# smdogroup/eigd

Measured on AMD Instinct MI355X. Metric: adjoint_mode_derivatives_per_sec, higher is better.
Workload: dtype f64

## Files before the change

### eigd_amd/_ffi.py

```python

import ctypes as C
import os

import numpy as np

_HERE = os.path.dirname(os.path.abspath(__file__))
LIB_PATH = os.environ.get("EIGD_LIB") or os.path.join(_HERE, "lib", "libeigd_hip.so")

EIGD_E_INVALID, EIGD_E_HIP, EIGD_E_NOTSPD, EIGD_E_INTERNAL = -1, -2, -3, -4


class EigdHipError(RuntimeError):
    """HIP runtime / device failure inside libeigd_hip.so."""


class NotPositiveDefiniteError(np.linalg.LinAlgError):
    """The shifted matrix handed to SpLuOperator is not positive definite."""


_lib = None

c_int, c_i64, c_dbl, c_sz, c_vp = C.c_int, C.c_int64, C.c_double, C.c_size_t, C.c_void_p
P = C.POINTER

# ... 52 lines not shown
    "eigd_project_stats": [c_vp, c_vp],
    "eigd_svqb_step": [c_vp, c_int, c_int, c_vp, c_int, c_vp, c_int, c_vp, c_int, c_vp, c_int],
    "eigd_project_to": [c_vp, c_int, c_int, c_int, c_vp, c_int, c_vp, c_int, c_vp, c_int, c_vp, c_int, c_dbl, c_vp, c_vp],
    "eigd_coldot_dev": [c_vp, c_int, c_int, c_vp, c_int, c_vp, c_int, c_vp],
    "eigd_coldot": [c_vp, c_int, c_int, c_vp, c_int, c_vp, c_int, c_vp],
    "eigd_coldot_dd": [c_vp, c_int, c_int, c_vp, c_int, c_vp, c_int, c_vp],
    "eigd_lincomb": [c_vp, c_int, c_int, c_vp, c_int, c_int, c_vp, c_vp, c_vp],
    "eigd_stack_dot": [c_vp, c_int, c_int, c_int, c_vp, c_i64, c_int, c_vp, c_int, c_vp],
    "eigd_stack_axpy": [c_vp, c_int, c_int, c_int, c_vp, c_i64, c_int, c_vp, c_vp, c_int, c_dbl],
    "eigd_stack_axpy_dot": [c_vp, c_int, c_int, c_int, c_vp, c_i64, c_int, c_vp, c_vp, c_int, c_dbl, c_vp],
    "eigd_stack_cgs2": [c_vp, c_int, c_int, c_int, c_vp, c_i64, c_int, c_vp, c_int, c_dbl, c_vp, c_vp],
    "eigd_stack_cgs2_pair": [c_vp, c_int, c_int, c_int, c_vp, c_i64, c_int, c_vp, c_int, c_dbl, c_vp, c_vp],
    "eigd_pair_orthonormalise": [c_vp, c_int, c_int, c_vp, c_int, c_vp, c_vp, c_int, c_vp, c_int, c_vp, c_vp],
    "eigd_csr_update_values_dev": [c_vp, c_vp],
    "eigd_factor_refactor_dev": [c_vp, c_vp],
    "eigd_assembler_create": [c_vp, c_int, c_int, c_int, c_vp, c_vp],
    "eigd_assembler_free": [c_vp],
    "eigd_assembler_nnz": [c_vp, c_vp],
    "eigd_assembler_pattern": [c_vp, c_vp, c_vp],
    "eigd_assemble": [c_vp, c_vp, c_int, c_vp, c_vp, c_vp],
    "eigd_elem_linear_matrices": [c_vp, c_int, c_int, c_vp, c_vp, c_int, c_vp, c_vp, c_vp],
    "eigd_colnorm2_dev": [c_vp, c_int, c_int, c_vp, c_int, c_vp],
    "eigd_colnorm2_fetch": [c_vp, c_vp, c_int],
    "eigd_colnorm2_publish": [c_vp, c_vp, c_int],
    "eigd_scale_inv_norm": [c_vp, c_int, c_int, c_vp, c_int, c_vp, c_int, c_vp, c_vp],
    "eigd_copy_block": [c_vp, c_int, c_int, c_vp, c_int, c_vp, c_int],
    "eigd_cg_state_rows": [],
    "eigd_cg_coefficients": [c_vp, c_int, c_int, c_vp, c_int, c_vp, c_int, c_vp, c_int, c_vp, c_vp, c_int, c_int, c_vp],
    "eigd_cg_solution_coefficients": [c_vp, c_int, c_vp, c_int, c_vp],
    "eigd_stack_axpy_dev": [c_vp, c_int, c_int, c_int, c_vp, c_i64, c_int, c_vp, c_vp, c_int, c_dbl],
    "eigd_spmm_cg": [c_vp, c_vp, c_int, c_vp, c_int, c_vp, c_int, c_vp, c_int, c_vp, c_vp, c_int, c_int, c_vp],
    "eigd_cg_update": [c_vp, c_int, c_int, c_vp, c_int, c_vp, c_int, c_vp, c_int, c_vp, c_int, c_vp, c_int, c_vp, c_int, c_vp,
                       c_int, c_vp],
    "eigd_gather_cols": [c_vp, c_int, c_int, c_vp, c_int, c_vp, c_vp, c_int],
    "eigd_scatter_cols": [c_vp, c_int, c_int, c_vp, c_int, c_vp, c_vp, c_int],
    "eigd_elem_bilinear": [c_vp, c_int, c_int, c_vp, c_vp, c_int, c_vp, c_vp, c_vp, c_int, c_vp, c_int, c_int, c_dbl,
                           c_vp],
    "eigd_elem_linear_adjoint": [c_vp, c_int, c_int, c_vp, c_int, c_vp, c_vp, c_vp, c_vp, c_int, c_vp, c_int, c_int,
                                 c_dbl, c_vp],
    "eigd_design_map": [c_vp, c_i64, c_int, c_dbl, c_dbl, c_dbl, c_vp, c_vp, c_vp],
    "eigd_comm_unique_id": [c_vp],
    "eigd_comm_init": [c_vp, c_int, c_int, c_vp, P(c_vp)],
    "eigd_comm_destroy": [c_vp],
    "eigd_comm_info": [c_vp, P(c_int), P(c_int)],
    "eigd_allreduce_sum": [c_vp, c_vp, c_i64],
    "eigd_allreduce_max": [c_vp, c_vp, c_i64],
}
EXPORTED = sorted(list(_SIGNATURES) + ["eigd_last_error"])


def lib():
    global _lib
    if _lib is None:
        if not os.path.exists(LIB_PATH):
            raise EigdHipError(
                f"{LIB_PATH} not found: build it with `make -C eigd_amd/csrc` "
                "(or __graft_entry__.build()); eigd_amd has no CPU fallback"
            )
        L = C.CDLL(LIB_PATH)
        L.eigd_last_error.restype = C.c_char_p
        L.eigd_last_error.argtypes = []
        for name, args in _SIGNATURES.items():
            fn = getattr(L, name, None)
            if fn is None:
                if os.environ.get("EIGD_LIB"):
                    continue
# ... 29 lines not shown
```

### eigd_amd/adjoint.py

```python

import numpy as np

from . import tuning
from .device import writable_result
from .operators import DeviceOperator, FactorApply, SpLuOperator

MODES = ("normal", "buckling")


def _check_mode(mode):
    if mode not in MODES:
        raise ValueError(f"Unknown mode {mode!r}")


def _is_close(a, b, atol=1e-5):
    return bool(np.fabs(a - b) < atol)


def are_eigenvalues_repeated(lam, atol=1e-5):
    return any(_is_close(lam[i], lam[i + 1], atol) for i in range(len(lam) - 1))


class DeviceProblem:
    def __init__(self, ctx, A, B, factor, mode):
# ... 22 lines not shown
        self.Phi = Phi_dev if Phi_dev is not None else self.ctx.from_host(Phi_host)
        self.BPhi = self.opB.apply(self.Phi)
        self._uscale = {}
        self._rebuild_deflation()

    def set_extra(self, Phix_dev, lam_x):
        self.Phix, self.lam_x = Phix_dev, (None if lam_x is None else np.asarray(lam_x, dtype=float))
        self.BPhix = None if Phix_dev is None else self.opB.apply(Phix_dev)
        self._rebuild_deflation()

    def _rebuild_deflation(self):
        self.PhiD = self.BPhiD = None
        self._uscale.pop("D", None)
        if self.Phix is None or self.Phi is None or self.Phix.k == 0:
            return
        if np.max(np.abs(self.BPhix.tdot(self.Phi))) > 1e-9:
            return
        N, nx = self.Phi.k, self.Phix.k
        self.PhiD, self.BPhiD = self.ctx.empty(self.n, N + nx), self.ctx.empty(self.n, N + nx)
        for dst, a, b in ((self.PhiD, self.Phi, self.Phix), (self.BPhiD, self.BPhi, self.BPhix)):
            dst.cols(0, N).copy_from(a)
            dst.cols(N, N + nx).copy_from(b)

    def _projector(self):
        if self.use_extra and self.PhiD is not None:
            return self.BPhiD, self.PhiD
        return self.BPhi, self.Phi

    def project_r(self, X):
        U, V = self._projector()
        return X.project(U, V)

    def project_r_norm2(self, X, tol=0.0, requested_only=False):
        U, V = (self.BPhi, self.Phi) if requested_only else self._projector()
        which = "D" if U is self.BPhiD else "N"
        if self._uscale.get(which) is None:
            self._uscale[which] = float(np.max(U.colnorms()))
        return X.project_norm2(U, V, uscale=self._uscale[which], tol=tol)

    def project_s(self, X):
        U, V = self._projector()
        return X.project(V, U)

    def extra_correction_coefficients(self, dPhib, lam, Gx=None):
        if Gx is None:
            Gx = -self.Phix.tdot(dPhib)
        if self.mode != "normal":
            Gx = self.lam_x[:, None] * Gx
        return Gx / (self.lam_x[:, None] - np.asarray(lam, dtype=float)[None, :])

    def adjoint_operator(self, X, lam_cols, out=None):
        tA = self.opA.apply(X)
        tB = self.opB.apply(X)
        out = self.ctx.empty(X.n, X.k) if out is None else out
        if self.mode == "normal":
            return out.assign_lincomb([(1.0, tA), (-np.asarray(lam_cols), tB)])
        return out.assign_lincomb([(1.0, tB), (np.asarray(lam_cols), tA)])

    def residual(self, Phib, psi, lam_cols):
        tA = self.opA.apply(psi)
        tB = self.opB.apply(psi)
        R = self.ctx.empty(psi.n, psi.k)
        lam_cols = np.asarray(lam_cols)
        if self.mode == "normal":
            return R.assign_lincomb([(-1.0, Phib), (-1.0, tA), (lam_cols, tB)])
        return R.assign_lincomb([(-1.0, Phib), (-1.0, tB), (-lam_cols, tA)])


def _default_factor(A, B, lam, sigma, mode, ctx):
    if sigma is None:
        sigma = 0.9 * lam[0]
# ... 755 lines not shown
    if np.isfinite(g):
        proj_every = int(max(1, min(4, np.floor(np.log(1e6) / np.log(max(4.0 * g, 1.0 + 1e-12))))))
    if tuning.cg_projection_period:
        proj_every = int(tuning.cg_projection_period)
    LAST_ROUND["cg_projection_period"] = proj_every
    LAST_ROUND["cg_solution"] = "from the z history" if deferred else "recurrence"

    def sptr(lo):
        return state.cols(lo, 64).ptr

    def zslab(j):
        if not deferred:
            return z
        q, i = divmod(j - 1, _CG_CHUNK)
        while len(zchunks) <= q:
            zchunks.append(ctx.workspace_stack(("cg_z", len(zchunks), n, k), _CG_CHUNK, n, k))
        return zchunks[q][i]

    if deferred:
        shapes = ctx.__dict__.setdefault("_cg_z_shapes", [])
        if (n, k) in shapes:
            shapes.remove((n, k))
        shapes.append((n, k))
        for old in shapes[:-2]:
            for tag in [t for t in ctx.__dict__.get("_ws", {}) if isinstance(t, tuple) and t[0] == "cg_z" and t[2:] == old]:
                del ctx.__dict__["_ws"][tag]
        del shapes[:-2]

    norms_of = {}

    def project_in(j):
        return j % proj_every == 0 or j >= maxsteps

    def first_part(j, lo, hi, n2, n2_lo):
        nonlocal r, r_old, psi, psi_old
        kk = hi - lo
        try:
            zj = zslab(j)
        except _ffi.EigdHipError:
            failed.append(j)
            return
        rv, zv, yv = r.cols(lo, hi), zj.cols(lo, hi), y.cols(lo, hi)
        prob.fac.apply_to(rv, zv, count=0)
        n2p = None if n2 is None else n2.cols(lo - n2_lo, hi - n2_lo).ptr
        logp = log.cols(lo, 64).ptr if deferred else None
        if tuning.cg_dots_in_spmm:
            call("eigd_spmm_cg", ctx.h, Kop.csr.h, kk, zv.ptr, zv.ld, yv.ptr, yv.ld, rv.ptr, rv.ld, n2p, sptr(lo), int(j),
                 1 if j == 1 else 0, logp)
        else:
            Kop.apply(zv, yv)
            call("eigd_cg_coefficients", ctx.h, n, kk, zv.ptr, zv.ld, rv.ptr, rv.ld, yv.ptr, yv.ld, n2p, sptr(lo), int(j),
                 1 if j == 1 else 0, logp)
        rov = r_old.cols(lo, hi)
        own = None if project_in(j) else ctx.empty(1, kk)
        if deferred:
            call("eigd_cg_update", ctx.h, n, kk, rv.ptr, rv.ld, rov.ptr, rov.ld, None, 0, None, 0, None, 0,
                 yv.ptr, yv.ld, sptr(lo), 1 if j == 1 else 0, own.ptr if own is not None else None)
        else:
            psv, pov = psi.cols(lo, hi), psi_old.cols(lo, hi)
            call("eigd_cg_update", ctx.h, n, kk, rv.ptr, rv.ld, rov.ptr, rov.ld, psv.ptr, psv.ld, pov.ptr, pov.ld, zv.ptr,
                 zv.ld, yv.ptr, yv.ld, sptr(lo), 1 if j == 1 else 0, own.ptr if own is not None else None)
            psi, psi_old = psi_old, psi
        norms_of[j] = own
        r, r_old = r_old, r

    lo, hi = _active_range(done)
    first_part(1, lo, hi, None, lo)
    if host_work is not None:
        host_work()
    rng_j = (lo, hi)
    nsteps = 0
    j = 1
    while True:
        lo, hi = rng_j
        if _CG_TRACE_HOOK is not None:
            _CG_TRACE_HOOK(prob, j, r.cols(lo, hi), lo, hi, project_in(j))
        if project_in(j):
            if j > 1 and proj_every > 1 and tuning.cg_project_previous:
                prob.project_r_norm2(r_old.cols(lo, hi), tol=proj_tol, requested_only=not tuning.cg_project_extra_pairs)
            n2 = prob.project_r_norm2(r.cols(lo, hi), tol=proj_tol, requested_only=not tuning.cg_project_extra_pairs)
        else:
            n2 = norms_of[j]
            call("eigd_colnorm2_publish", ctx.h, n2.ptr, hi - lo)
        norms_of.pop(j - 1, None)
        nsteps = j
        live = np.flatnonzero(~done)
        expect_all = tuning.predict_finish and j > 1 and all(
            len(hist[c]) >= 2 and hist[c][-2] > 0.0 and hist[c][-1] * min(hist[c][-1] / hist[c][-2], 1.0) < 4.0 * tol
            for c in live)
        nxt = _active_range(done)
        in_flight = False
        if j < maxsteps and not expect_all:
            first_part(j + 1, nxt[0], nxt[1], n2, lo)
            in_flight = True
        norms2 = ctx.fetch_colnorm2(hi - lo)
        for c in range(lo, hi):
            if done[c]:
                continue
            hist[c].append(float(np.sqrt(max(norms2[c - lo], 0.0))))
            if norms2[c - lo] < tol2:
                info[c] = j
                done[c] = converged[c] = True
        if failed:
            break
        for c in np.flatnonzero(~done):
            h = hist[c]
            frozen = len(h) >= 3 and h[-1] > 0.0 and abs(h[-1] - h[-2]) <= 1e-14 * h[-1] and abs(h[-2] - h[-3]) <= 1e-14 * h[-2]
            if frozen or (len(h) > 12 and not h[-1] < 0.5 * h[-11]):
                gave_up.append(int(c))
        if gave_up:
# ... 610 lines not shown
```

### eigd_amd/csrc/common.h

```cpp
#pragma once
#include <hip/hip_runtime.h>

#include <cstdarg>
#include <cstdint>
#include <cstdio>
#include <string>
#include <vector>

#include "../../include/eigd_hip.h"

namespace eigd {

void set_error(const char* fmt, ...);
const char* get_error();

#define EIGD_HIP(call)                                                                           \
  do {                                                                                           \
    hipError_t _e = (call);                                                                      \
    if (_e != hipSuccess) {                                                                      \
      ::eigd::set_error("%s failed: %s (%s:%d)", #call, hipGetErrorString(_e), __FILE__, __LINE__); \
      return EIGD_E_HIP;                                                                         \
    }                                                                                            \
  } while (0)

#define EIGD_REQUIRE(cond, ...)      \
  do {                               \
    if (!(cond)) {                   \
      ::eigd::set_error(__VA_ARGS__); \
      return EIGD_E_INVALID;         \
    }                                \
  } while (0)

#define EIGD_LAUNCH_CHECK() EIGD_HIP(hipGetLastError())

constexpr int kThreads = 256;
constexpr int kMaxK = 64;

inline int next_pow2(int v) {
  int p = 1;
  while (p < v) p <<= 1;
  return p;
}

}

struct eigd_ctx {
  int device = 0;
  hipStream_t stream = nullptr;
  hipEvent_t ev0 = nullptr, ev1 = nullptr;
  double* scratch = nullptr;
  size_t scratch_bytes = 0;
  double* coef = nullptr;
  size_t coef_bytes = 0;
  int n_cu = 256;
  double* pinned = nullptr;
  hipEvent_t ev_pinned = nullptr;
  int pinned_count = 0;
  void* bounce = nullptr;
  double* pinned_h = nullptr;
  size_t pinned_h_bytes = 0;
  int* proj_stats = nullptr;

  int ensure_scratch(size_t bytes);
  int ensure_coef(size_t bytes);
};

namespace eigd {
int publish_norm2(eigd_ctx* ctx, const double* dOut, int k);
int cg_coefficients_from_partials(eigd_ctx* ctx, const double* partial, int nblocks, int k, const double* dNorm2,
                                  double* dState, int step, int first, double* dLog);
// ... 2 lines not shown
```

### eigd_amd/csrc/dense.hip

```cpp
#include <algorithm>

#include <cmath>
#include <cstdlib>
#include <cstdint>
#include <cstring>
#include <vector>
#include <type_traits>

#include "common.h"

namespace eigd {

constexpr int kRB = 64;
constexpr int kMaxBlocks = 1024;

static inline int grid_for_rows(int n, int rows_per_block) {
  int64_t need = (static_cast<int64_t>(n) + rows_per_block - 1) / rows_per_block;
  return static_cast<int>(std::max<int64_t>(1, std::min<int64_t>(need, kMaxBlocks)));
}

__global__ __launch_bounds__(kThreads) void reduce_partials_kernel(const double* __restrict__ partial, int nblocks,
                                                                  int nout, double* __restrict__ out,
                                                                  const int* __restrict__ gate = nullptr) {
  if (gate != nullptr && *gate == 0) return;
// ... 649 lines not shown
      const int b = tb * 16 + li;
      double outv[4];
#pragma unroll
      for (int reg = 0; reg < 4; ++reg)
        outv[reg] = (beta == 0.0) ? alpha * accs[tb][reg] : beta * xv[tb][reg] + alpha * accs[tb][reg];
#pragma unroll
      for (int reg = 0; reg < 4; ++reg) {
        const int r = lk + 4 * reg;
        if (r < rows && b < kx) {
          X[(base + r) * ldx + b] = outv[reg];
          nsq[tb] += outv[reg] * outv[reg];
        }
      }
    }
  }
  if (normpart != nullptr) {
#pragma unroll
    for (int tb = 0; tb < 4; ++tb) {
      double v = nsq[tb];
      v += __shfl_xor(v, 16, 64);
      v += __shfl_xor(v, 32, 64);
      if (lk == 0) nred[wave][tb * 16 + li] = v;
    }
    __syncthreads();
    if (tid < kx) {
      double v = 0.0;
#pragma unroll
      for (int w = 0; w < kThreads / 64; ++w) v += nred[w][tid];
      normpart[static_cast<int64_t>(blockIdx.x) * kx + tid] = v;
    }
  }
}

constexpr int kPanelW = 64, kPanelsMax = 3, kPanelOutMax = 80, kPanelThreads = 512;

template <int NP>
__global__ __launch_bounds__(kPanelThreads) void gemm_nn_panels_kernel(int n, int ku, int kx, const double* __restrict__ U,
                                                                       int64_t pstride, const double* __restrict__ C, int ldc,
                                                                       int c0, double* __restrict__ Out, int64_t ostride,
                                                                       int o0, int opw, int old) {
  extern __shared__ double Cs[];
  const int tid = threadIdx.x;
  const int cld = kx + 16;
  for (int e = tid; e < NP * kPanelW * cld; e += kPanelThreads) {
    const int slot = e / cld, b = e - slot * cld;
    const int p = slot >> 6, sl = slot & 63;
    const int k = kPanelW * p + 16 * (sl & 3) + (sl >> 2);
    Cs[e] = (k < ku && b < kx) ? C[static_cast<int64_t>(k) * ldc + c0 + b] : 0.0;
  }
  __syncthreads();
  const int wave = tid >> 6, lane = tid & 63;
  const int li = lane & 15, lk = lane >> 4;
  const int ntb = (kx + 15) >> 4;
  const int64_t ngroups = (static_cast<int64_t>(n) + 15) / 16;
  const int64_t gstride = static_cast<int64_t>(gridDim.x) * (kPanelThreads / 64);
  auto fetch = [&](int p, int64_t base, int rows, double (&a)[16]) {
    const double* up = U + p * pstride + (base + li) * kPanelW + 16 * lk;
    const int left = ku - (kPanelW * p + 16 * lk);
    if (li < rows && left >= 16) {
      const double2_t* vp = reinterpret_cast<const double2_t*>(up);
#pragma unroll
      for (int q = 0; q < 8; ++q) {
        const double2_t v = vp[q];
        a[2 * q] = v.x;
        a[2 * q + 1] = v.y;
      }
// ... 358 lines not shown
  EIGD_REQUIRE(n > 0 && ku >= 1 && ku <= 2 * kMaxK && kx >= 1 && kx <= kMaxK && ldx >= kx && ldu >= ku && ldv >= ku,
               "bad shape n=%d ku=%d kx=%d", n, ku, kx);
  EIGD_REQUIRE(tol >= 0.0, "tol = relative size of an update that matters (0: the default, 1e-13)");
  const double skip_tol = tol > 0.0 ? tol : 1e-13;
  constexpr bool measured = true;
  const int nbd = grid_for_rows(n, 64);
  int rc = ctx->ensure_scratch(sizeof(double) * (static_cast<size_t>(kMaxK) * kx + static_cast<size_t>(nbd) * kx));
  if (rc) return rc;
  rc = project_coefficients(ctx, n, ku, kx, dV, ldv, dX, ldx, measured ? dOut : nullptr);
  if (rc) return rc;
  int* gate = nullptr;
  if (measured) {
    gate = reinterpret_cast<int*>(ctx->coef + static_cast<size_t>(ku) * kx);
    if (!ctx->proj_stats) {
      EIGD_HIP(hipMalloc(reinterpret_cast<void**>(&ctx->proj_stats), 2 * sizeof(int)));
      EIGD_HIP(hipMemsetAsync(ctx->proj_stats, 0, 2 * sizeof(int), ctx->stream));
    }
    hipLaunchKernelGGL(project_decide_kernel, dim3(1), dim3(kThreads), 0, ctx->stream, ctx->coef, ku, kx, dOut,
                       uscale > 0.0 ? skip_tol / uscale : skip_tol, gate, ctx->proj_stats);
    EIGD_LAUNCH_CHECK();
  }
  double* normpart = ctx->scratch + static_cast<size_t>(kMaxK) * kx;
  int nparts = 0;
  for (int a0 = 0; a0 < ku; a0 += kMaxK) {
    const int ka = std::min(kMaxK, ku - a0);
    const bool last = a0 + kMaxK >= ku;
    rc = gemm_nn_device(ctx, n, ka, kx, dU + a0, ldu, 1, ctx->coef + static_cast<size_t>(a0) * kx, dX, ldx, -1.0, 1.0,
                        last ? normpart : nullptr, last ? &nparts : nullptr, gate);
    if (rc) return rc;
  }
  rc = reduce_to_host(ctx, normpart, nparts, kx, dOut, nullptr, gate);
  if (rc) return rc;
  return publish_norm2(ctx, dOut, kx);
}

int eigd_project_to(eigd_ctx* ctx, int n, int ku, int kx, const double* dU, int ldu, const double* dV, int ldv, double* dX,
                    int ldx, double* dC, int ldc, double tol, double* dFlag, const double* dNorm2) {
  EIGD_REQUIRE(ctx && dU && dV && dX && dC, "null argument");
  EIGD_REQUIRE(n > 0 && ku >= 1 && ku <= kMaxK && kx >= 1 && kx <= kMaxK && ldx >= kx && ldu >= ku && ldv >= ku && ldc >= kx,
               "bad shape n=%d ku=%d kx=%d", n, ku, kx);
  EIGD_REQUIRE(tol >= 0.0 && (tol == 0.0 || dFlag != nullptr), "a measured update needs somewhere to report to");
  const bool measured = tol > 0.0;
  int rc = ctx->ensure_coef(sizeof(double) * (static_cast<size_t>(ku) * kx + 8 + kMaxK));
  if (rc) return rc;
  double* norms = ctx->coef + static_cast<size_t>(ku) * kx + 8;
  double* coef = (ldc == kx) ? dC : ctx->coef;
  rc = project_coefficients(ctx, n, ku, kx, dV, ldv, dX, ldx, (measured && dNorm2 == nullptr) ? norms : nullptr, coef);
  if (rc) return rc;
  if (coef != dC)
    EIGD_HIP(hipMemcpy2DAsync(dC, sizeof(double) * ldc, ctx->coef, sizeof(double) * kx, sizeof(double) * kx, ku,
                              hipMemcpyDeviceToDevice, ctx->stream));
  int* gate = nullptr;
  if (measured) {
    gate = reinterpret_cast<int*>(ctx->coef + static_cast<size_t>(ku) * kx);
    hipLaunchKernelGGL(project_decide_kernel, dim3(1), dim3(kThreads), 0, ctx->stream, coef, ku, kx,
                       dNorm2 != nullptr ? dNorm2 : norms, tol, gate, static_cast<int*>(nullptr), dFlag);
    EIGD_LAUNCH_CHECK();
  }
  return gemm_nn_device(ctx, n, ku, kx, dU, ldu, 1, coef, dX, ldx, -1.0, 1.0, nullptr, nullptr, gate);
}

int eigd_svqb_step(eigd_ctx* ctx, int n, int p, double* dX, int ldx, double* dBX, int ldbx, double* dC, int first,
                   double* dFlag, int update_bx) {
  EIGD_REQUIRE(ctx && dX && dBX && dC && dFlag, "null argument");
  EIGD_REQUIRE(n > 0 && p >= 1 && p <= kSvqbMax && ldx >= p && ldbx >= p, "bad shape n=%d p=%d (blocks of at most %d)", n, p,
               kSvqbMax);
// ... 483 lines not shown
```

### eigd_amd/csrc/krylov.hip

```cpp
#include <algorithm>
#include <cstdint>
#include <type_traits>

#include "common.h"

namespace eigd {

enum CgRow { kRr = 0, kGam = 1, kRho = 2, kDone = 3, kTol2 = 4, kAlpha = 5, kSteps = 6, kFlag = 7, kGamNow = 8, kRhoNow = 9,
             kBadRr = 10, kBadDen = 11, kBadStep = 12,
             kCgRows = 13 };

constexpr int kCgMaxBlocks = 1024;

static inline int cg_grid(int n, int rows_per_block) {
  const int64_t need = (static_cast<int64_t>(n) + rows_per_block - 1) / rows_per_block;
  return static_cast<int>(std::max<int64_t>(1, std::min<int64_t>(need, kCgMaxBlocks)));
}

__device__ __forceinline__ double wave_sum_partials(const double* __restrict__ partial, int nblocks, int nout, int o) {
  const int lane = threadIdx.x & 63;
  double s = 0.0;
  int g = lane;
  for (; g + 7 * 64 < nblocks; g += 8 * 64) {
    double v[8];
#pragma unroll
    for (int q = 0; q < 8; ++q) v[q] = partial[static_cast<int64_t>(g + 64 * q) * nout + o];
#pragma unroll
    for (int q = 0; q < 8; ++q) s += v[q];
  }
  for (; g < nblocks; g += 64) s += partial[static_cast<int64_t>(g) * nout + o];
#pragma unroll
  for (int off = 32; off > 0; off >>= 1) s += __shfl_down(s, off, 64);
  return __shfl(s, 0, 64);
}

template <int KP>
__global__ __launch_bounds__(kThreads) void cg_dots_kernel(int n, int k, const double* __restrict__ Z, int ldz,
                                                          const double* __restrict__ R, int ldr,
                                                          const double* __restrict__ Y, int ldy,
                                                          double* __restrict__ partial) {
  constexpr int RP = kThreads / KP;
  __shared__ double red[kThreads];
  const int c = threadIdx.x % KP, rr = threadIdx.x / KP;
// ... 244 lines not shown
```

### eigd_amd/device.py

```python

import contextlib
import ctypes as C

import numpy as np

from . import _ffi
from ._ffi import c_vp, call, hptr

_default_ctx = None


class Context:

    def __init__(self, device=0, _parent=None):
        h = c_vp()
        if _parent is None:
            call("eigd_ctx_create", int(device), C.byref(h))
        else:
            call("eigd_ctx_fork", _parent.h, C.byref(h))
        self.h = h
        self.device = int(device)
        self.parent = _parent

    def fork(self, index=0):
# ... 524 lines not shown
            return self.add_product(U, t, alpha=-1.0, beta=1.0)
        call("eigd_project", self.ctx.h, self.n, U.k, self.k, U.ptr, U.ld, V.ptr, V.ld, self.ptr, self.ld)
        return self

    def project_to(self, U, V, Cdev, tol=0.0, flag=None, norm2=None):
        if U.k > 64 or self.k > 64 or (Cdev.n, Cdev.k) != (U.k, self.k):
            raise ValueError("project_to: panels of at most 64 columns, coefficient block U.k x self.k")
        if norm2 is not None and norm2.n * norm2.k != self.k:
            raise ValueError("project_to: one squared norm per column of the block")
        call("eigd_project_to", self.ctx.h, self.n, U.k, self.k, U.ptr, U.ld, V.ptr, V.ld, self.ptr, self.ld, Cdev.ptr,
             Cdev.ld, float(tol), flag.ptr if flag is not None else None, norm2.ptr if norm2 is not None else None)
        return self

    def coldot_dev(self, other, out):
        if self.k > 64 or (other.n, other.k) != (self.n, self.k) or out.n * out.k != self.k:
            raise ValueError("coldot_dev: blocks of the same shape with at most 64 columns, one result per column")
        call("eigd_coldot_dev", self.ctx.h, self.n, self.k, self.ptr, self.ld, other.ptr, other.ld, out.ptr)
        return out

    def svqb_step(self, BX, Cdev, first, flag, update_bx=True):
        if self.k > 32 or (BX.n, BX.k) != (self.n, self.k) or (Cdev.n, Cdev.k) != (self.k, self.k) or Cdev.ld != self.k:
            raise ValueError("svqb_step: blocks of at most 32 columns, a contiguous p x p coefficient block")
        call("eigd_svqb_step", self.ctx.h, self.n, self.k, self.ptr, self.ld, BX.ptr, BX.ld, Cdev.ptr, 1 if first else 0,
             flag.ptr, 1 if update_bx else 0)
        return self

    def project_norm2(self, U, V, uscale=0.0, tol=0.0):
        if U.k > 128 or self.k > 64:
            return self.project(U, V).colnorm2_dev()
        out = self.ctx.empty(1, self.k)
        call("eigd_project_norm2", self.ctx.h, self.n, U.k, self.k, U.ptr, U.ld, V.ptr, V.ld, self.ptr, self.ld, out.ptr,
             float(uscale), float(tol))
        return out

    def gather_cols(self, cols):
        cols = np.ascontiguousarray(cols, dtype=np.int32)
        out = self.ctx.empty(self.n, len(cols))
        for c0 in range(0, len(cols), 64):
            c1 = min(len(cols), c0 + 64)
            sub = np.ascontiguousarray(cols[c0:c1])
            call("eigd_gather_cols", self.ctx.h, self.n, c1 - c0, self.ptr, self.ld, hptr(sub),
                 out.cols(c0, c1).ptr, out.ld)
        return out

    def gather_cols_into(self, dst, cols):
        cols = np.ascontiguousarray(cols, dtype=np.int32)
        if (dst.n, dst.k) != (self.n, len(cols)):
            raise ValueError("shape mismatch in column gather")
        for c0 in range(0, len(cols), 64):
            c1 = min(len(cols), c0 + 64)
            sub = np.ascontiguousarray(cols[c0:c1])
            call("eigd_gather_cols", self.ctx.h, self.n, c1 - c0, self.ptr, self.ld, hptr(sub),
                 dst.cols(c0, c1).ptr, dst.ld)
        return dst

    def scatter_cols_into(self, dst, cols):
        cols = np.ascontiguousarray(cols, dtype=np.int32)
        for c0 in range(0, len(cols), 64):
            c1 = min(len(cols), c0 + 64)
            sub = np.ascontiguousarray(cols[c0:c1])
            call("eigd_scatter_cols", self.ctx.h, self.n, c1 - c0, self.cols(c0, c1).ptr, self.ld, hptr(sub),
                 dst.ptr, dst.ld)
        return dst


class DeviceStack:
# ... 719 lines not shown
```

### eigd_amd/tuning.py

```python

recurrence = "auto"
cg_solution_from_history = True
cg_dots_in_spmm = True
cg_projection_period = 0
cg_projection_tol = 1e-11
cg_project_previous = True
cg_project_extra_pairs = False
steps_per_pass = 2
inner_projections = False
pair_defect_tol = 1e-10
predict_finish = True
reorth_tol = 1e-13

host_twins = "returned"

iram_block = 0
iram_extra = None
iram_basis = 0
iram_basis_factor = 2.5
iram_extra_tol = 1e-11
iram_seed = 12345
lanczos_local_first_pass = True
lanczos_fused_restart = True
deflate_extra = True
laa_internal = True
laa_relation = True
```

### include/eigd_hip.h

```cpp
#ifndef EIGD_HIP_H
#define EIGD_HIP_H

#include <stddef.h>
#include <stdint.h>

#ifdef __cplusplus
extern "C" {
#endif

#define EIGD_OK 0
#define EIGD_E_INVALID (-1)
#define EIGD_E_HIP (-2)
#define EIGD_E_NOTSPD (-3)
#define EIGD_E_INTERNAL (-4)

typedef struct eigd_ctx eigd_ctx;
typedef struct eigd_mat eigd_mat;
typedef struct eigd_symbolic eigd_symbolic;
typedef struct eigd_factor eigd_factor;
typedef struct eigd_lane eigd_lane;

const char* eigd_last_error(void);
int eigd_version(void);

// ... 73 lines not shown
int eigd_coldot(eigd_ctx* ctx, int n, int k, const double* dX, int ldx, const double* dY, int ldy, double* hout);
int eigd_coldot_dev(eigd_ctx* ctx, int n, int k, const double* dX, int ldx, const double* dY, int ldy, double* dOut);
int eigd_coldot_dd(eigd_ctx* ctx, int n, int k, const double* dX, int ldx, const double* dY, int ldy, double* hout);
int eigd_lincomb(eigd_ctx* ctx, int n, int k, double* dOut, int ldo, int nterms, const double* const* dXs,
                 const int* ldxs, const double* hcoef);
int eigd_stack_dot(eigd_ctx* ctx, int n, int k, int ns, const double* dS, int64_t slab, int lds, const double* dT,
                   int ldt, double* hH);
int eigd_stack_axpy(eigd_ctx* ctx, int n, int k, int ns, const double* dS, int64_t slab, int lds, const double* hH,
                    double* dT, int ldt, double alpha);
int eigd_stack_axpy_dev(eigd_ctx* ctx, int n, int k, int ns, const double* dS, int64_t slab, int lds, const double* dH,
                        double* dT, int ldt, double alpha);
int eigd_stack_axpy_dot(eigd_ctx* ctx, int n, int k, int ns, const double* dS, int64_t slab, int lds, const double* hH1,
                        double* dT, int ldt, double alpha, double* hH2);
int eigd_stack_cgs2(eigd_ctx* ctx, int n, int k, int ns, const double* dS, int64_t slab, int lds, double* dT, int ldt,
                    double tol, double* hH, int* hpasses);
int eigd_stack_cgs2_pair(eigd_ctx* ctx, int n, int k, int ns, const double* dS, int64_t slab, int lds, double* dT, int ldt,
                         double tol, double* hH, int* hpasses);
int eigd_pair_orthonormalise(eigd_ctx* ctx, int n, int k, double* dT, int ldt, const double* dNorm2, double* dW1, int ldw1,
                             double* dW2, int ldw2, const unsigned char* hskip, double* dOut);
int eigd_colnorm2_dev(eigd_ctx* ctx, int n, int k, const double* dX, int ldx, double* dOut);
int eigd_colnorm2_fetch(eigd_ctx* ctx, double* hout, int k);
int eigd_colnorm2_publish(eigd_ctx* ctx, const double* dNorm2, int k);
int eigd_scale_inv_norm(eigd_ctx* ctx, int n, int k, const double* dX, int ldx, double* dOut, int ldo,
                        const double* dNorm2, const unsigned char* hskip);
int eigd_cg_state_rows(void);
int eigd_cg_coefficients(eigd_ctx* ctx, int n, int k, const double* dZ, int ldz, const double* dR, int ldr, const double* dY,
                         int ldy, const double* dNorm2, double* dState, int step, int first, double* dLog);
int eigd_spmm_cg(eigd_ctx* ctx, eigd_mat* A, int k, const double* dZ, int ldz, double* dY, int ldy, const double* dR, int ldr,
                 const double* dNorm2, double* dState, int step, int first, double* dLog);
int eigd_cg_solution_coefficients(eigd_ctx* ctx, int k, const double* dLog, int nsteps, double* dS);
int eigd_cg_update(eigd_ctx* ctx, int n, int k, const double* dR, int ldr, double* dRold, int ldro, const double* dPsi,
                   int ldpsi, double* dPsiOld, int ldpso, const double* dZ, int ldz, const double* dY, int ldy,
                   const double* dState, int first, double* dNorm2);
int eigd_copy_block(eigd_ctx* ctx, int n, int k, const double* dSrc, int lds, double* dDst, int ldd);
int eigd_gather_cols(eigd_ctx* ctx, int n, int kdst, const double* dSrc, int lds, const int32_t* hcols, double* dDst,
                     int ldd);
int eigd_scatter_cols(eigd_ctx* ctx, int n, int ksrc, const double* dSrc, int lds, const int32_t* hcols, double* dDst,
                      int ldd);

int eigd_elem_bilinear(eigd_ctx* ctx, int nelem, int nd, const int32_t* d_edofs, const double* dMe, int per_elem,
                       const int32_t* d_etype, const double* dscale, const double* dW, int ldw, const double* dV, int ldv,
                       int k, double alpha, double* dOut);

typedef struct eigd_assembler eigd_assembler;
int eigd_assembler_create(eigd_ctx* ctx, int n, int nelem, int nd, const int32_t* elem_dofs, eigd_assembler** out);
int eigd_assembler_free(eigd_assembler* a);
int eigd_assembler_nnz(eigd_assembler* a, int64_t* nnz);
int eigd_assembler_pattern(eigd_assembler* a, int32_t* hindptr , int32_t* hindices );
int eigd_assemble(eigd_assembler* a, const double* dMe, int per_elem, const int32_t* d_etype, const double* dscale,
                  double* dvals);
int eigd_elem_linear_matrices(eigd_ctx* ctx, int nelem, int nd, const int32_t* d_edofs, const double* du, int nterms,
                              const double* dL, const double* dQ, double* dOut);

int eigd_elem_linear_adjoint(eigd_ctx* ctx, int nelem, int nd, const int32_t* d_edofs, int nterms, const double* dL,
                             const double* dQ, const double* dscale, const double* dW, int ldw, const double* dV,
                             int ldv, int k, double alpha, double* dOut);

int eigd_design_map(eigd_ctx* ctx, int64_t n, int kind, double p, double c0, double c1, const double* dx,
                    const double* dg, double* dout);

#define EIGD_COMM_ID_BYTES 128
typedef struct eigd_comm eigd_comm;
int eigd_comm_unique_id(void* hid128);
int eigd_comm_init(eigd_ctx* ctx, int nranks, int rank, const void* hid128, eigd_comm** out);
int eigd_comm_destroy(eigd_comm* comm);
int eigd_comm_info(eigd_comm* comm, int* nranks, int* rank);
// ... 8 lines not shown
```

Before: 681.8.

## Fuse CG residual update with deflation projection of both residual blocks

Adds a fused kernel that applies the CG residual update and, in the same pass over the rows, computes the projection coefficients and norms for both the old and the new residual. A paired MFMA kernel then subtracts the projections from both blocks. The aim is to avoid separate passes (update, then project r_old, then project r) that each reread the n-by-k blocks and launch their own kernels. It adds a large new code path with extra shared memory and register pressure, and it only runs when the deferred and projection conditions hold.

```diff
diff --git a/eigd_amd/_ffi.py b/eigd_amd/_ffi.py
--- a/eigd_amd/_ffi.py
+++ b/eigd_amd/_ffi.py
@@ -108,6 +108,8 @@
     "eigd_spmm_cg": [c_vp, c_vp, c_int, c_vp, c_int, c_vp, c_int, c_vp, c_int, c_vp, c_vp, c_int, c_int, c_vp],
     "eigd_cg_update": [c_vp, c_int, c_int, c_vp, c_int, c_vp, c_int, c_vp, c_int, c_vp, c_int, c_vp, c_int, c_vp, c_int, c_vp,
                        c_int, c_vp],
+    "eigd_cg_update_project": [c_vp, c_int, c_int, c_vp, c_int, c_vp, c_int, c_vp, c_int, c_vp, c_int, c_int, c_vp, c_int,
+                               c_vp, c_int, c_vp, c_vp, c_dbl, c_dbl],
     "eigd_gather_cols": [c_vp, c_int, c_int, c_vp, c_int, c_vp, c_vp, c_int],
     "eigd_scatter_cols": [c_vp, c_int, c_int, c_vp, c_int, c_vp, c_vp, c_int],
     "eigd_elem_bilinear": [c_vp, c_int, c_int, c_vp, c_vp, c_int, c_vp, c_vp, c_vp, c_int, c_vp, c_int, c_int, c_dbl,
diff --git a/eigd_amd/adjoint.py b/eigd_amd/adjoint.py
--- a/eigd_amd/adjoint.py
+++ b/eigd_amd/adjoint.py
@@ -78,11 +78,15 @@
         return X.project(U, V)
 
     def project_r_norm2(self, X, tol=0.0, requested_only=False):
+        U, V, uscale = self.residual_projector(requested_only)
+        return X.project_norm2(U, V, uscale=uscale, tol=tol)
+
+    def residual_projector(self, requested_only=False):
         U, V = (self.BPhi, self.Phi) if requested_only else self._projector()
         which = "D" if U is self.BPhiD else "N"
         if self._uscale.get(which) is None:
             self._uscale[which] = float(np.max(U.colnorms()))
-        return X.project_norm2(U, V, uscale=self._uscale[which], tol=tol)
+        return U, V, self._uscale[which]
 
     def project_s(self, X):
         U, V = self._projector()
@@ -904,6 +908,15 @@
     def project_in(j):
         return j % proj_every == 0 or j >= maxsteps
 
+    projected_in_update = set()
+
+    def fused_projector(j):
+        if not (deferred and tuning.cg_fused_projection and project_in(j) and j > 1 and proj_every > 1
+                and tuning.cg_project_previous and _CG_TRACE_HOOK is None):
+            return None
+        U, V, uscale = prob.residual_projector(requested_only=not tuning.cg_project_extra_pairs)
+        return (U, V, uscale) if U.k <= 64 else None
+
     def first_part(j, lo, hi, n2, n2_lo):
         nonlocal r, r_old, psi, psi_old
         kk = hi - lo
@@ -925,7 +938,11 @@
                  1 if j == 1 else 0, logp)
         rov = r_old.cols(lo, hi)
         own = None if project_in(j) else ctx.empty(1, kk)
-        if deferred:
+        panels = fused_projector(j)
+        if panels is not None:
+            own = rv.cg_update_project(rov, yv, sptr(lo), 0, panels[0], panels[1], uscale=panels[2], tol=proj_tol)[1]
+            projected_in_update.add(j)
+        elif deferred:
             call("eigd_cg_update", ctx.h, n, kk, rv.ptr, rv.ld, rov.ptr, rov.ld, None, 0, None, 0, None, 0,
                  yv.ptr, yv.ld, sptr(lo), 1 if j == 1 else 0, own.ptr if own is not None else None)
         else:
@@ -947,7 +964,10 @@
         lo, hi = rng_j
         if _CG_TRACE_HOOK is not None:
             _CG_TRACE_HOOK(prob, j, r.cols(lo, hi), lo, hi, project_in(j))
-        if project_in(j):
+        if j in projected_in_update:
+            n2 = norms_of[j]
+            call("eigd_colnorm2_publish", ctx.h, n2.ptr, hi - lo)
+        elif project_in(j):
             if j > 1 and proj_every > 1 and tuning.cg_project_previous:
                 prob.project_r_norm2(r_old.cols(lo, hi), tol=proj_tol, requested_only=not tuning.cg_project_extra_pairs)
             n2 = prob.project_r_norm2(r.cols(lo, hi), tol=proj_tol, requested_only=not tuning.cg_project_extra_pairs)
diff --git a/eigd_amd/csrc/common.h b/eigd_amd/csrc/common.h
--- a/eigd_amd/csrc/common.h
+++ b/eigd_amd/csrc/common.h
@@ -36,6 +36,10 @@
 constexpr int kThreads = 256;
 constexpr int kMaxK = 64;
 
+enum CgRow { kRr = 0, kGam = 1, kRho = 2, kDone = 3, kTol2 = 4, kAlpha = 5, kSteps = 6, kFlag = 7, kGamNow = 8, kRhoNow = 9,
+             kBadRr = 10, kBadDen = 11, kBadStep = 12,
+             kCgRows = 13 };
+
 inline int next_pow2(int v) {
   int p = 1;
   while (p < v) p <<= 1;
diff --git a/eigd_amd/csrc/dense.hip b/eigd_amd/csrc/dense.hip
--- a/eigd_amd/csrc/dense.hip
+++ b/eigd_amd/csrc/dense.hip
@@ -705,6 +705,240 @@
   }
 }
 
+template <int KW>
+__global__ __launch_bounds__(kThreads) void cg_update_project_kernel(int n, int ku, int kx, const double* __restrict__ r,
+                                                                    int ldr, double* __restrict__ ro, int ldro,
+                                                                    const double* __restrict__ y, int ldy,
+                                                                    const double* __restrict__ state, int first,
+                                                                    const double* __restrict__ V, int64_t rsv,
+                                                                    double* __restrict__ partial_r,
+                                                                    double* __restrict__ partial_n,
+                                                                    double* __restrict__ xnorm_part_r,
+                                                                    double* __restrict__ xnorm_part_n) {
+  constexpr int ROWS = kTsElems / KW;
+  constexpr int RPT = kThreads / KW;
+  constexpr int HALF = ROWS / 2;
+  constexpr int HELEMS = kTsElems / 2;
+  constexpr int IT = HELEMS / kThreads;
+  constexpr int TPW = (KW == 32) ? 1 : 4;
+  __shared__ double Vs[HELEMS];
+  __shared__ double Rs[HELEMS];
+  __shared__ double Ns[HELEMS];
+  double rsq = 0.0, nsq = 0.0;
+  const int tid = threadIdx.x, wave = tid >> 6, lane = tid & 63;
+  const int li = lane & 15, lk = lane >> 4;
+  const int nta = (ku + 15) >> 4, ntb = (kx + 15) >> 4;
+  const int ntiles = nta * ntb;
+  const int col = tid % KW, row0 = tid / KW;
+  const bool live = col < kx;
+  const double gam = live ? state[kGamNow * kMaxK + col] : 0.0, rho = live ? state[kRhoNow * kMaxK + col] : 1.0;
+  const double al = live ? state[kAlpha * kMaxK + col] : 0.0;
+  const bool moves = gam != 0.0;
+  const bool three = moves && !first && rho != 1.0;
+  double4_t accr[TPW], accn[TPW];
+#pragma unroll
+  for (int t = 0; t < TPW; ++t) accr[t] = accn[t] = double4_t{0.0, 0.0, 0.0, 0.0};
+  double fv[IT], fr[IT], fy[IT], fo[IT];
+  auto fetch = [&](int64_t base) {
+#pragma unroll
+    for (int it = 0; it < IT; ++it) {
+      const int64_t row = base + row0 + RPT * it;
+      const bool in = row < n && live;
+      fv[it] = *((row < n && col < ku) ? V + row * rsv + col : &g_zero_word);
+      fr[it] = *(in ? r + row * ldr + col : &g_zero_word);
+      fy[it] = *((in && moves) ? y + row * ldy + col : &g_zero_word);
+      fo[it] = *((in && three) ? ro + row * ldro + col : &g_zero_word);
+    }
+  };
+  const int64_t stride = static_cast<int64_t>(gridDim.x) * ROWS;
+  int64_t chunk = static_cast<int64_t>(blockIdx.x) * ROWS;
+  if (chunk < n) fetch(chunk);
+  for (; chunk < n; chunk += stride) {
+#pragma unroll
+    for (int h = 0; h < 2; ++h) {
+      const int64_t base = chunk + h * HALF;
+      __syncthreads();
+#pragma unroll
+      for (int it = 0; it < IT; ++it) {
+        const int64_t row = base + row0 + RPT * it;
+        const double rv = fr[it];
+        double rn = rv;
+        if (moves) {
+          const double yv = fy[it];
+          rn = rv - gam * (rv - al * yv);
+          if (three) rn = rho * rn + (1.0 - rho) * fo[it];
+        }
+        if (row < n && live)
+          ro[row * ldro + col] = rn;
+        else
+          rn = 0.0;
+        Vs[(row0 + RPT * it) * KW + col] = fv[it];
+        Rs[(row0 + RPT * it) * KW + col] = rv;
+        Ns[(row0 + RPT * it) * KW + col] = rn;
+        rsq += rv * rv;
+        nsq += rn * rn;
+      }
+      __syncthreads();
+      if (h == 0)
+        fetch(base + HALF);
+      else if (chunk + stride < n)
+        fetch(chunk + stride);
+#pragma unroll
+      for (int t = 0; t < TPW; ++t) {
+        const int tile = wave + 4 * t;
+        if (tile < ntiles) {
+          const int ta = tile / ntb, tb = tile - ta * ntb;
+          double4_t cr = accr[t], cn = accn[t];
+#pragma unroll
+          for (int q = 0; q < HALF / 4; ++q) {
+            const double a = Vs[(4 * q + lk) * KW + 16 * ta + li];
+            cr = __builtin_amdgcn_mfma_f64_16x16x4f64(a, Rs[(4 * q + lk) * KW + 16 * tb + li], cr, 0, 0, 0);
+            cn = __builtin_amdgcn_mfma_f64_16x16x4f64(a, Ns[(4 * q + lk) * KW + 16 * tb + li], cn, 0, 0, 0);
+          }
+          accr[t] = cr;
+          accn[t] = cn;
+        }
+      }
+    }
+  }
+  double* pr = partial_r + static_cast<int64_t>(blockIdx.x) * ku * kx;
+  double* pn = partial_n + static_cast<int64_t>(blockIdx.x) * ku * kx;
+#pragma unroll
+  for (int t = 0; t < TPW; ++t) {
+    const int tile = wave + 4 * t;
+    if (tile >= ntiles) break;
+    const int ta = tile / ntb, tb = tile - ta * ntb;
+#pragma unroll
+    for (int reg = 0; reg < 4; ++reg) {
+      const int a = ta * 16 + lk + 4 * reg, b = tb * 16 + li;
+      if (a < ku && b < kx) {
+        pr[a * kx + b] = accr[t][reg];
+        pn[a * kx + b] = accn[t][reg];
+      }
+    }
+  }
+  __syncthreads();
+  Rs[row0 * KW + col] = rsq;
+  Ns[row0 * KW + col] = nsq;
+  __syncthreads();
+  if (tid < kx) {
+    double vr = 0.0, vn = 0.0;
+#pragma unroll
+    for (int q = 0; q < RPT; ++q) {
+      vr += Rs[q * KW + tid];
+      vn += Ns[q * KW + tid];
+    }
+    xnorm_part_r[static_cast<int64_t>(blockIdx.x) * kx + tid] = vr;
+    xnorm_part_n[static_cast<int64_t>(blockIdx.x) * kx + tid] = vn;
+  }
+}
+
+template <int NQ>
+__global__ __launch_bounds__(kThreads) void gemm_nn_direct_pair_kernel(int n, int ku, int kx, const double* __restrict__ U,
+                                                                      int64_t rsu, const double* __restrict__ C0,
+                                                                      const double* __restrict__ C1,
+                                                                      double* __restrict__ X0, int ldx0,
+                                                                      double* __restrict__ X1, int ldx1,
+                                                                      double* __restrict__ normpart0,
+                                                                      double* __restrict__ normpart1,
+                                                                      const int* __restrict__ gates) {
+  const bool on[2] = {gates[0] != 0, gates[1] != 0};
+  if (!on[0] && !on[1]) return;
+  extern __shared__ double Cs[];
+  __shared__ double nred[2][kThreads / 64][64];
+  double nsq[2][4] = {{0.0, 0.0, 0.0, 0.0}, {0.0, 0.0, 0.0, 0.0}};
+  const int tid = threadIdx.x;
+  const int cld = cs_stride(kx);
+  const double* const Cg[2] = {C0, C1};
+  double* const Xg[2] = {X0, X1};
+  const int ldx[2] = {ldx0, ldx1};
+  for (int q = tid; q < 4 * NQ * kx; q += kThreads) {
+    const int slot = q / kx, b = q % kx;
+    const int k = NQ * (slot & 3) + (slot >> 2);
+#pragma unroll
+    for (int s = 0; s < 2; ++s) Cs[(s * 4 * NQ + slot) * cld + b] = (k < ku && on[s]) ? Cg[s][k * kx + b] : 0.0;
+  }
+  __syncthreads();
+  const int wave = tid >> 6, lane = tid & 63;
+  const int li = lane & 15, lk = lane >> 4;
+  const int ntb = (kx + 15) >> 4;
+  const int64_t ngroups = (static_cast<int64_t>(n) + 15) / 16;
+  const int64_t gstride = static_cast<int64_t>(gridDim.x) * 4;
+  const bool vec = (ku == 4 * NQ) && ((rsu & 1) == 0) && ((reinterpret_cast<uintptr_t>(U) & 15) == 0);
+  for (int64_t g = static_cast<int64_t>(blockIdx.x) * 4 + wave; g < ngroups; g += gstride) {
+    const int64_t base = g * 16;
+    const int rows = static_cast<int>((n - base) < 16 ? (n - base) : 16);
+    const double* up = U + (base + li) * rsu + NQ * lk;
+    double a[NQ];
+    if (vec && rows == 16) {
+      const double2_t* vp = reinterpret_cast<const double2_t*>(up);
+#pragma unroll
+      for (int q = 0; q < NQ / 2; ++q) {
+        const double2_t v = vp[q];
+        a[2 * q] = v.x;
+        a[2 * q + 1] = v.y;
+      }
+    } else {
+#pragma unroll
+      for (int q = 0; q < NQ; ++q) a[q] = *((li < rows && NQ * lk + q < ku) ? up + q : &g_zero_word);
+    }
+    double xv[2][4][4];
+#pragma unroll
+    for (int s = 0; s < 2; ++s)
+#pragma unroll
+      for (int tb = 0; tb < 4; ++tb)
+#pragma unroll
+        for (int reg = 0; reg < 4; ++reg) {
+          const int r = lk + 4 * reg, b = tb * 16 + li;
+          xv[s][tb][reg] = *((on[s] && tb < ntb && r < rows && b < kx) ? Xg[s] + (base + r) * ldx[s] + b : &g_zero_word);
+        }
+#pragma unroll
+    for (int s = 0; s < 2; ++s) {
+      if (!on[s]) continue;
+#pragma unroll
+      for (int tb = 0; tb < 4; ++tb) {
+        if (tb >= ntb) break;
+        const int b = tb * 16 + li;
+        double4_t acc = double4_t{0.0, 0.0, 0.0, 0.0};
+#pragma unroll
+        for (int q = 0; q < NQ; ++q) {
+          const double bv = (b < kx) ? Cs[(s * 4 * NQ + 4 * q + lk) * cld + b] : 0.0;
+          acc = __builtin_amdgcn_mfma_f64_16x16x4f64(a[q], bv, acc, 0, 0, 0);
+        }
+#pragma unroll
+        for (int reg = 0; reg < 4; ++reg) {
+          const int r = lk + 4 * reg;
+          const double outv = xv[s][tb][reg] - acc[reg];
+          if (r < rows && b < kx) {
+            Xg[s][(base + r) * ldx[s] + b] = outv;
+            nsq[s][tb] += outv * outv;
+          }
+        }
+      }
+    }
+  }
+#pragma unroll
+  for (int s = 0; s < 2; ++s)
+#pragma unroll
+    for (int tb = 0; tb < 4; ++tb) {
+      double v = nsq[s][tb];
+      v += __shfl_xor(v, 16, 64);
+      v += __shfl_xor(v, 32, 64);
+      if (lk == 0) nred[s][wave][tb * 16 + li] = v;
+    }
+  __syncthreads();
+  if (tid < kx) {
+#pragma unroll
+    for (int s = 0; s < 2; ++s) {
+      if (!on[s]) continue;
+      double v = 0.0;
+#pragma unroll
+      for (int w = 0; w < kThreads / 64; ++w) v += nred[s][w][tid];
+      (s == 0 ? normpart0 : normpart1)[static_cast<int64_t>(blockIdx.x) * kx + tid] = v;
+    }
+  }
+}
+
 constexpr int kPanelW = 64, kPanelsMax = 3, kPanelOutMax = 80, kPanelThreads = 512;
 
 template <int NP>
@@ -1129,6 +1363,62 @@
   rc = reduce_to_host(ctx, normpart, nparts, kx, dOut, nullptr, gate);
   if (rc) return rc;
   return publish_norm2(ctx, dOut, kx);
+}
+
+int eigd_cg_update_project(eigd_ctx* ctx, int n, int k, double* dR, int ldr, double* dRold, int ldro, const double* dY,
+                           int ldy, const double* dState, int first, int ku, const double* dU, int ldu, const double* dV,
+                           int ldv, double* dNorm2R, double* dNorm2New, double uscale, double tol) {
+  EIGD_REQUIRE(ctx && dR && dRold && dY && dState && dU && dV && dNorm2R && dNorm2New, "null argument");
+  EIGD_REQUIRE(uscale >= 0.0 && tol >= 0.0, "uscale and tol as in eigd_project_norm2");
+  EIGD_REQUIRE(n > 0 && k >= 1 && k <= kMaxK && ku >= 1 && ku <= kMaxK && ldr >= k && ldro >= k && ldy >= k && ldu >= ku &&
+                   ldv >= ku,
+               "bad shape n=%d k=%d ku=%d", n, k, ku);
+  const double skip_tol = tol > 0.0 ? tol : 1e-13;
+  const int nb = grid_for_rows(n, kRB), nbd = grid_for_rows(n, 64);
+  const size_t nout = static_cast<size_t>(ku) * k;
+  int rc = ctx->ensure_coef(sizeof(double) * (2 * nout + 8));
+  if (rc) return rc;
+  rc = ctx->ensure_scratch(sizeof(double) * (2 * nb * nout + 2 * static_cast<size_t>(nb) * k + 2 * static_cast<size_t>(nbd) * k));
+  if (rc) return rc;
+  double* coef[2] = {ctx->coef, ctx->coef + nout};
+  int* gates = reinterpret_cast<int*>(ctx->coef + 2 * nout);
+  double* part[2] = {ctx->scratch, ctx->scratch + nb * nout};
+  double* xpart[2] = {part[1] + nb * nout, part[1] + nb * nout + static_cast<size_t>(nb) * k};
+  double* normpart[2] = {xpart[1] + static_cast<size_t>(nb) * k, xpart[1] + static_cast<size_t>(nb) * k + static_cast<size_t>(nbd) * k};
+  double* norm2[2] = {dNorm2R, dNorm2New};
+  if (!ctx->proj_stats) {
+    EIGD_HIP(hipMalloc(reinterpret_cast<void**>(&ctx->proj_stats), 2 * sizeof(int)));
+    EIGD_HIP(hipMemsetAsync(ctx->proj_stats, 0, 2 * sizeof(int), ctx->stream));
+  }
+  if (ku <= 32 && k <= 32)
+    hipLaunchKernelGGL(cg_update_project_kernel<32>, dim3(nb), dim3(kThreads), 0, ctx->stream, n, ku, k, dR, ldr, dRold, ldro,
+                       dY, ldy, dState, first, dV, static_cast<int64_t>(ldv), part[0], part[1], xpart[0], xpart[1]);
+  else
+    hipLaunchKernelGGL(cg_update_project_kernel<64>, dim3(nb), dim3(kThreads), 0, ctx->stream, n, ku, k, dR, ldr, dRold, ldro,
+                       dY, ldy, dState, first, dV, static_cast<int64_t>(ldv), part[0], part[1], xpart[0], xpart[1]);
+  EIGD_LAUNCH_CHECK();
+  for (int s = 0; s < 2; ++s) {
+    rc = reduce_to_host(ctx, part[s], nb, static_cast<int>(nout), coef[s], nullptr);
+    if (rc) return rc;
+    rc = reduce_to_host(ctx, xpart[s], nb, k, norm2[s], nullptr);
+    if (rc) return rc;
+    hipLaunchKernelGGL(project_decide_kernel, dim3(1), dim3(kThreads), 0, ctx->stream, coef[s], ku, k, norm2[s],
+                       uscale > 0.0 ? skip_tol / uscale : skip_tol, gates + s, ctx->proj_stats);
+    EIGD_LAUNCH_CHECK();
+  }
+  const size_t cbytes = sizeof(double) * 2 * (ku <= 32 ? 32 : 64) * ((k % 32 == 0) ? k + 16 : k);
+  if (ku <= 32)
+    hipLaunchKernelGGL(gemm_nn_direct_pair_kernel<8>, dim3(nbd), dim3(kThreads), cbytes, ctx->stream, n, ku, k, dU,
+                       static_cast<int64_t>(ldu), coef[0], coef[1], dR, ldr, dRold, ldro, normpart[0], normpart[1], gates);
+  else
+    hipLaunchKernelGGL(gemm_nn_direct_pair_kernel<16>, dim3(nbd), dim3(kThreads), cbytes, ctx->stream, n, ku, k, dU,
+                       static_cast<int64_t>(ldu), coef[0], coef[1], dR, ldr, dRold, ldro, normpart[0], normpart[1], gates);
+  EIGD_LAUNCH_CHECK();
+  for (int s = 0; s < 2; ++s) {
+    rc = reduce_to_host(ctx, normpart[s], nbd, k, norm2[s], nullptr, gates + s);
+    if (rc) return rc;
+  }
+  return EIGD_OK;
 }
 
 int eigd_project_to(eigd_ctx* ctx, int n, int ku, int kx, const double* dU, int ldu, const double* dV, int ldv, double* dX,
diff --git a/eigd_amd/csrc/krylov.hip b/eigd_amd/csrc/krylov.hip
--- a/eigd_amd/csrc/krylov.hip
+++ b/eigd_amd/csrc/krylov.hip
@@ -5,10 +5,6 @@
 #include "common.h"
 
 namespace eigd {
-
-enum CgRow { kRr = 0, kGam = 1, kRho = 2, kDone = 3, kTol2 = 4, kAlpha = 5, kSteps = 6, kFlag = 7, kGamNow = 8, kRhoNow = 9,
-             kBadRr = 10, kBadDen = 11, kBadStep = 12,
-             kCgRows = 13 };
 
 constexpr int kCgMaxBlocks = 1024;
 
diff --git a/eigd_amd/device.py b/eigd_amd/device.py
--- a/eigd_amd/device.py
+++ b/eigd_amd/device.py
@@ -580,6 +580,12 @@
         call("eigd_project_norm2", self.ctx.h, self.n, U.k, self.k, U.ptr, U.ld, V.ptr, V.ld, self.ptr, self.ld, out.ptr,
              float(uscale), float(tol))
         return out
+
+    def cg_update_project(self, r_old, y, state_ptr, first, U, V, uscale=0.0, tol=0.0):
+        n2r, n2n = self.ctx.empty(1, self.k), self.ctx.empty(1, self.k)
+        call("eigd_cg_update_project", self.ctx.h, self.n, self.k, self.ptr, self.ld, r_old.ptr, r_old.ld, y.ptr, y.ld,
+             state_ptr, int(first), U.k, U.ptr, U.ld, V.ptr, V.ld, n2r.ptr, n2n.ptr, float(uscale), float(tol))
+        return n2r, n2n
 
     def gather_cols(self, cols):
         cols = np.ascontiguousarray(cols, dtype=np.int32)
diff --git a/eigd_amd/tuning.py b/eigd_amd/tuning.py
--- a/eigd_amd/tuning.py
+++ b/eigd_amd/tuning.py
@@ -5,6 +5,7 @@
 cg_projection_period = 0
 cg_projection_tol = 1e-11
 cg_project_previous = True
+cg_fused_projection = True
 cg_project_extra_pairs = False
 steps_per_pass = 2
 inner_projections = False
diff --git a/include/eigd_hip.h b/include/eigd_hip.h
--- a/include/eigd_hip.h
+++ b/include/eigd_hip.h
@@ -129,6 +129,9 @@
 int eigd_cg_update(eigd_ctx* ctx, int n, int k, const double* dR, int ldr, double* dRold, int ldro, const double* dPsi,
                    int ldpsi, double* dPsiOld, int ldpso, const double* dZ, int ldz, const double* dY, int ldy,
                    const double* dState, int first, double* dNorm2);
+int eigd_cg_update_project(eigd_ctx* ctx, int n, int k, double* dR, int ldr, double* dRold, int ldro, const double* dY,
+                           int ldy, const double* dState, int first, int ku, const double* dU, int ldu, const double* dV,
+                           int ldv, double* dNorm2R, double* dNorm2New, double uscale, double tol);
 int eigd_copy_block(eigd_ctx* ctx, int n, int k, const double* dSrc, int lds, double* dDst, int ldd);
 int eigd_gather_cols(eigd_ctx* ctx, int n, int kdst, const double* dSrc, int lds, const int32_t* hcols, double* dDst,
                      int ldd);
```

Result: no change. 692.0 (median of 6 runs) (+1.5%).
